# epeters13/pyCuSDR

Hardware: AMD Instinct MI355X
Metric: IQ Msamples/sec through Doppler matched-filter bank (256 bins, 2^20 chunk) (higher is better)
Workload: dtype f32

## Files before the change

__graft_entry__.py:

```python
import os
import subprocess
import sys

ROOT = os.path.dirname(os.path.abspath(__file__))
if ROOT not in sys.path:
    sys.path.insert(0, ROOT)

SRC = os.path.join(ROOT, 'pycusdr_amd', 'csrc', 'mfbank.hip')
CSRC = os.path.join(ROOT, 'pycusdr_amd', 'csrc')
DEPS = [SRC] + sorted(os.path.join(CSRC, h) for h in os.listdir(CSRC) if h.endswith(('.hpp', '.h'))) + [os.path.join(ROOT, 'include', 'mfbank.h')]
LIB = os.path.join(ROOT, 'pycusdr_amd', 'libmfbank.so')


HASHFILE = LIB + '.srchash'


def _src_hash():
    import hashlib
    h = hashlib.sha256()
    for d in DEPS:
        h.update(open(d, 'rb').read())
    return h.hexdigest()


def _stale():
    if not os.path.exists(LIB):
        return True
    try:
        return open(HASHFILE).read().strip() != _src_hash()
    except OSError:
        return True


def build(force=False):
    if force or _stale():
        import fcntl
        with open(LIB + '.lock', 'w') as lock:
            fcntl.flock(lock, fcntl.LOCK_EX)
            if force or _stale():
                hipcc = os.environ.get('HIPCC', '/opt/rocm/bin/hipcc')
                tmp = f'{LIB}.tmp.{os.getpid()}'
                cmd = [hipcc, '--offload-arch=gfx950', '-O3', '-std=c++17', '-shared', '-fPIC', '-pthread',
                       '-Wall', '-Wextra', '-Wno-unused-parameter', '-o', tmp, SRC]
                print('[build]', ' '.join(cmd), flush=True)
                subprocess.check_call(cmd, cwd=ROOT)
                os.replace(tmp, LIB)
                with open(HASHFILE, 'w') as f:
                    f.write(_src_hash())
    import pycusdr_amd
    from pycusdr_amd import _lib
    _lib.load()
    return LIB


def smoke():
    import numpy as np
    build()
    from pycusdr_amd import config as cfg, signals as sg
    from pycusdr_amd.protocol import loadProtocol
    from pycusdr_amd.demodulator import UHF
    from oracle import mfbank_oracle as orc

    bs, ov = 15, 1 << 10
    N = 1 << bs
    conf = cfg.bench_config('bench_GMSK', blockSize=bs, doppCarrierSteps=32)
    proto = loadProtocol('bench_GMSK')(conf=conf)
    demod = UHF.Demodulator(conf, proto, 'UHF-H')
    sig = sg.s1_stream(2, N, ov, 'GMSK', snr_db=20.0, seed=1)
    raw = demod.get_signalBufferHostPointer()
    raw[:] = sig[(N - ov):(N - ov) + N]
    fo, metric, _, snr = demod.uploadAndFindCarrier(raw)
    scores = demod.bank.get_scores()
    X = demod.bank.get_spectrum()
    bits, centres, trust, spSym = demod.demodulate()

    _, masks = proto.get_filter(N, 16, 3)
    ref = orc.doppler_scores(X, masks, demod.doppCyperSymNorm, True)
    rel = np.abs(scores - ref).max() / ref.max()
    assert rel < 1e-5, f'doppler scores differ from the oracle: {rel}'
    oidx, _ = orc.find_doppler_est(scores, demod.num_dopplers, 0, True)
    pick = orc.interpolate_doppler(oidx, demod.doppCyperSymNorm, demod.doppHzLUT, demod.centreFreqOffset)
    assert pick['dopplerIdxlast'] == int(demod.dopplerIdxlast) == N // 4, (pick, demod.dopplerIdxlast)
    xc = demod.bank.get_xcorr()
    ref_xc = orc.demod_xcorr(X, masks, int(demod.dopplerIdxlast))
    assert np.abs(xc - ref_xc).max() / np.abs(ref_xc).max() < 1e-5
    assert abs(spSym - 16.0) < 0.01 and len(bits) > 1900
    step = N - ov
    win = demod.blockWindows(2)[0]
    win[:] = sig[:2 * step + ov]
    demod.beginBlocks(0, 2)
    (_, rec0), (est1, rec1) = demod.endBlocks(0)
    assert est1[0] == fo and est1[3] == snr and rec1['spSym'] == spSym, (est1, fo, snr)
    raw[:] = sig[step:step + N]
    demod.uploadAndFindCarrier(raw)
    one = demod.demodulateDevice()
    assert np.array_equal(rec1['symbols'], one['symbols']) and np.array_equal(rec1['centres'], one['centres'])
    print(f'[smoke] ok: freq offset {fo:.1f} Hz, metric {metric:.2f}, SNR {snr:.1f} dB, spSym {spSym:.4f}, '
          f'{len(bits)} bits, score rel err {rel:.2e}; a batch of two blocks equals the blocks one by one')
    demod.close()


if __name__ == '__main__':
    build(force='--force' in sys.argv)
    if '--smoke' in sys.argv:
        smoke()
```

pycusdr_amd/csrc/wrap_kernels.hpp:

```cpp
#pragma once
#include "seg_kernels.hpp"

typedef _Float16 seg_h8 __attribute__((ext_vector_type(8)));
typedef float seg_f4 __attribute__((ext_vector_type(4)));

struct SegWArgs {
    SegFArgs f;
    const u32x4 *Wb;
    const int *Wexp;
    int T;
};

template <int PV, int KT>
struct SegWCfg {
    static constexpr int L = 256, PPL = 16, NT = 16, CT = 4;
    static constexpr int RT = PPL - PV;
    static constexpr int ND = RT + KT - 1;
    static constexpr int OFF = 16 * KT - 1;
    static constexpr int WSTR = 16 * (RT + KT);
    static_assert(RT >= 1 && RT + KT <= PPL, "the window is the first RT and the last KT register slots of a lane");
    static constexpr int WAVES = 1;
    static constexpr size_t lds_bytes() {
        return (size_t)SegCfg<256>::LDS_ELEMS * sizeof(cf) + (size_t)(SegCfg<256>::BLOCK / 64) * CT * WSTR * sizeof(cf);
    }
};

template <int KT>
struct SegWBin {
    seg_h8 hi[KT], lo[KT];
    cf q[8];
};

template <int PV, int KT>
DEVI void segw_body(const SegWArgs &w, const int blk) {
    static_assert(MFB_FFT_FUSED, "the fused 256-point transform");
    using Cfg = SegCfg<256>;
    using WC = SegWCfg<PV, KT>;
    constexpr int L = 256, NT = Cfg::NT, CT = Cfg::CT, PPL = Cfg::PPL, RT = WC::RT, ND = WC::ND, OFF = WC::OFF, WSTR = WC::WSTR;
    static_assert(NT == WC::NT && CT == WC::CT && PPL == WC::PPL, "256-point geometry");
    const SegFArgs &a = w.f;
    extern __shared__ __attribute__((aligned(16))) cf lds[];
    const int tid = threadIdx.x;
    const int wave = __builtin_amdgcn_readfirstlane(tid >> 6);
    const int lane = tid & 63;
    const int g = lane % NT;
    const int col = lane / NT;
    cf *mylds = lds + wave * Cfg::LDS_PER_TEAM + col * padlen(L);
    cf *wlds = lds + Cfg::LDS_ELEMS + wave * CT * WSTR;
    F256Regs f256;
    f256_setup(f256, a.twL + L, g);

    const int grp = blk % a.nsg;
    const int u = (blk / a.nsg) * (Cfg::BLOCK / 64) + wave;
    const int per_sc = a.nblk * a.nbc;
    const int sc = u / per_sc, rest = u - sc * per_sc;
    const int bk = rest / a.nbc, bc = rest - bk * a.nbc;
    const int gs0 = a.gbins ? 0 : (int)((long long)grp * a.nslots / a.nsg);
    const int glen = a.gbins ? a.nslots : (int)((long long)(grp + 1) * a.nslots / a.nsg) - gs0;
    const int gb0 = a.gbins ? (int)((long long)grp * a.dper / a.nsg) : 0;
    const int gblen = a.gbins ? (int)((long long)(grp + 1) * a.dper / a.nsg) - gb0 : a.dper;
    const int s0 = __builtin_amdgcn_readfirstlane(a.slot0 + gs0 + sc * a.fs);
    const int s1 = __builtin_amdgcn_readfirstlane(min(a.slot0 + gs0 + glen, s0 + a.fs));
    const int jb0 = __builtin_amdgcn_readfirstlane(gb0 + bc * a.fb);
    const int jb1 = __builtin_amdgcn_readfirstlane(min(gb0 + gblen, jb0 + a.fb));
    if (sc >= a.nsc || s0 >= s1 || jb0 >= jb1 || bk >= a.nblk) return;

    const unsigned nmask = (unsigned)a.N - 1u;
    const auto xr = mk_rsrc(a.x + (size_t)bk * (size_t)a.xstride, (unsigned)a.N * sizeof(cf));
    const auto qr = mk_rsrc(a.Qs, (unsigned)a.dper * (unsigned)(L * sizeof(float)));
    const auto br = mk_rsrc(w.Wb, (unsigned)a.dper * (unsigned)(KT * 2 * 64 * 16));
    auto load_q = [&](cf (&dst)[PPL / 2], int bin) {
#pragma unroll
        for (int jj = 0; jj < PPL / 4; ++jj)
            buf_load_cf2(qr, g * 4 * (int)sizeof(float), bin * (L * (int)sizeof(float)) + jj * NT * 4 * (int)sizeof(float), dst[2 * jj], dst[2 * jj + 1]);
    };
    auto load_b = [&](seg_h8 (&hi)[KT], seg_h8 (&lo)[KT], int bin) {
#pragma unroll
        for (int kk = 0; kk < KT; ++kk) {
            hi[kk] = __builtin_bit_cast(seg_h8, __builtin_amdgcn_raw_buffer_load_b128(br, lane * 16, (bin * KT + kk) * 2 * 1024, 0));
            lo[kk] = __builtin_bit_cast(seg_h8, __builtin_amdgcn_raw_buffer_load_b128(br, lane * 16, ((bin * KT + kk) * 2 + 1) * 1024, 0));
        }
    };
    constexpr int so_x = NT * (int)sizeof(cf);
    const int T = w.T;
    const int i16 = lane & 15, q = lane >> 4;
    const bool im_half = q >= 2;
    const int qo = 8 * (q & 1);

    const bool one_chunk = jb1 - jb0 <= 64;
    int wexl = jb0 + lane < jb1 ? w.Wexp[jb0 + lane] : 0;

    for (int slot = s0; slot < s1; ++slot) {
        cf v[PPL];
        {
            const unsigned e0 = (unsigned)(slot * CT + col) * (unsigned)a.V + (unsigned)g;
            const unsigned last = (unsigned)(slot * CT + CT - 1) * (unsigned)a.V + (unsigned)L;
            if (__builtin_amdgcn_readfirstlane(last <= (unsigned)a.N ? 1 : 0)) {
                const int vo_x = (int)(e0 * sizeof(cf));
#pragma unroll
                for (int i = 0; i < PPL; ++i) {
                    const cf t = buf_load_cf(xr, vo_x, i * so_x);
                    v[i] = mkc(t.y, t.x);
                }
            } else {
#pragma unroll
                for (int i = 0; i < PPL; ++i) {
                    const cf t = buf_load_cf(xr, (int)(((e0 + (unsigned)(NT * i)) & nmask) * sizeof(cf)), 0);
                    v[i] = mkc(t.y, t.x);
                }
            }
        }
        int ea;
        {
            cf *myw = wlds + col * WSTR;
            float mx = 0.f;
#pragma unroll
            for (int i = 0; i < RT; ++i) {
                const cf s = mkc(v[i].y, v[i].x);
                myw[g + NT * i + OFF] = s;
                mx = fmaxf(mx, fmaxf(fabsf(s.x), fabsf(s.y)));
            }
#pragma unroll
            for (int i = PPL - KT; i < PPL; ++i) {
                const int t = g + NT * i - L;
                const cf s = t >= -(T - 1) ? mkc(v[i].y, v[i].x) : mkc(0.f, 0.f);
                if (t + OFF >= 0) myw[t + OFF] = s;
                mx = fmaxf(mx, fmaxf(fabsf(s.x), fabsf(s.y)));
            }
#pragma unroll
            for (int m = 1; m < NT; m <<= 1) mx = fmaxf(mx, __shfl_xor(mx, m));
            int e;
            (void)frexpf(mx, &e);
            ea = 15 - e;
        }
        xsync<1>();
        cf A[PPL];
        {
            auto keep = [&](int, cf val, auto, auto nu) { A[decltype(nu)::value / NT] = val; };
            fft256_fused<0, PPL>(v, mylds, g, f256, keep);
        }
        cf pp[PPL / 2];
#pragma unroll
        for (int j = 0; j < PPL / 2; ++j) {
            const cf p0 = A[2 * j] * A[2 * j], p1 = A[2 * j + 1] * A[2 * j + 1];
            pp[j] = mkc(p0.x + p0.y, p1.x + p1.y);
        }
        seg_h8 ahi[CT][ND], alo[CT][ND];
        int eseg[CT];
#pragma unroll
        for (int c = 0; c < CT; ++c) {
            eseg[c] = __builtin_amdgcn_readlane(ea, NT * c);
            const cf *wc = wlds + c * WSTR;
#pragma unroll
            for (int di = 0; di < ND; ++di) {
                const int base = 16 * (di - (KT - 1)) + i16 - qo + OFF;
#pragma unroll
                for (int j = 0; j < 8; ++j) {
                    const cf s = wc[base - j];
                    const float sv = __builtin_ldexpf(im_half ? s.y : s.x, eseg[c]);
                    const _Float16 h = (_Float16)sv;
                    ahi[c][di][j] = h;
                    alo[c][di][j] = (_Float16)(sv - (float)h);
                }
            }
        }
        xsync<1>();

        for (int jc = jb0; jc < jb1; jc += 64) {
            if (!one_chunk) {
                wexl = jc + lane < jb1 ? w.Wexp[jc + lane] : 0;
                __builtin_amdgcn_s_waitcnt(0x0F70);
            }
            const int jc1 = min(jb1, jc + 64);
            SegWBin<KT> b0, b1;
            seg_f4 acc0[CT][RT], acc1[CT][RT];
            auto parseval = [&](const SegWBin<KT> &b) {
                cf t2[2] = {mkc(0.f, 0.f), mkc(0.f, 0.f)};
#pragma unroll
                for (int j = 0; j < PPL / 2; ++j) t2[j & 1] = __builtin_elementwise_fma(pp[j], b.q[j], t2[j & 1]);
                return (t2[0].x + t2[0].y) + (t2[1].x + t2[1].y);
            };
            auto fetch = [&](SegWBin<KT> &b, int bin) {
                load_q(b.q, bin);
                load_b(b.hi, b.lo, bin);
            };
            auto products = [&](seg_f4 (&acc)[CT][RT], const SegWBin<KT> &b) {
#pragma unroll
                for (int c = 0; c < CT; ++c) {
#pragma unroll
                    for (int rt = 0; rt < RT; ++rt) {
                        seg_f4 t = {0.f, 0.f, 0.f, 0.f};
#pragma unroll
                        for (int kk = 0; kk < KT; ++kk) {
                            const int di = rt - kk + KT - 1;
                            t = __builtin_amdgcn_mfma_f32_16x16x32_f16(alo[c][di], b.hi[kk], t, 0, 0, 0);
                            t = __builtin_amdgcn_mfma_f32_16x16x32_f16(ahi[c][di], b.lo[kk], t, 0, 0, 0);
                            t = __builtin_amdgcn_mfma_f32_16x16x32_f16(ahi[c][di], b.hi[kk], t, 0, 0, 0);
                        }
                        acc[c][rt] = t;
                    }
                }
            };
            auto finish = [&](const seg_f4 (&acc)[CT][RT], float tot, int jb) {
                const int wexp = __builtin_amdgcn_readlane(wexl, jb - jc);
                float wacc = 0.f;
#pragma unroll
                for (int c = 0; c < CT; ++c) {
                    float sq[RT];
#pragma unroll
                    for (int rt = 0; rt < RT; ++rt) {
                        const seg_f4 t = acc[c][rt];
                        sq[rt] = __builtin_fmaf(t.x, t.x, t.y * t.y) + __builtin_fmaf(t.z, t.z, t.w * t.w);
                    }
                    float s = sq[0];
#pragma unroll
                    for (int rt = 1; rt < RT; ++rt) s += sq[rt];
                    wacc += __builtin_ldexpf(s, wexp - 2 * eseg[c]);
                }
                float sv = __builtin_fmaf((float)L, tot, -wacc);
                sv += __int_as_float(__builtin_amdgcn_mov_dpp(__float_as_int(sv), 0xB1, 0xF, 0xF, true));
                sv += __int_as_float(__builtin_amdgcn_mov_dpp(__float_as_int(sv), 0x4E, 0xF, 0xF, true));
                sv += __int_as_float(__builtin_amdgcn_mov_dpp(__float_as_int(sv), 0x124, 0xF, 0xF, true));
                sv += __int_as_float(__builtin_amdgcn_mov_dpp(__float_as_int(sv), 0x128, 0xF, 0xF, true));
                const float r0 = __int_as_float(__builtin_amdgcn_readlane(__float_as_int(sv), 0));
                const float r1 = __int_as_float(__builtin_amdgcn_readlane(__float_as_int(sv), 16));
                const float r2 = __int_as_float(__builtin_amdgcn_readlane(__float_as_int(sv), 32));
                const float r3 = __int_as_float(__builtin_amdgcn_readlane(__float_as_int(sv), 48));
                return (r0 + r1) + (r2 + r3);
            };
            auto store = [&](float total, int jb) {
                if (lane < a.MU)
                    a.partials[((size_t)(a.part_row0 + bk * a.dper + jb) * a.MU + lane) * a.parts + slot] = lane == 0 ? total * a.scale : 0.f;
            };
            auto step = [&](seg_f4 (&accn)[CT][RT], SegWBin<KT> &bn, const seg_f4 (&accp)[CT][RT], SegWBin<KT> &bp, float totp, int jb) {
                const float totn = parseval(bn);
                fetch(bp, min(jb + 2, jc1 - 1));
                products(accn, bn);
                const float total = finish(accp, totp, jb);
#pragma unroll
                for (int i = 0; i < CT * RT * KT * 3; ++i) {
                    __builtin_amdgcn_sched_group_barrier(0x8, 1, 0);
                    __builtin_amdgcn_sched_group_barrier(0x2, 2, 0);
                }
                store(total, jb);
                return totn;
            };
            fetch(b0, jc);
            fetch(b1, min(jc + 1, jc1 - 1));
            float tot0 = parseval(b0), tot1 = 0.f;
            products(acc0, b0);
            int jb = jc;
            while (true) {
                if (jb + 1 >= jc1) {
                    store(finish(acc0, tot0, jb), jb);
                    break;
                }
                tot1 = step(acc1, b1, acc0, b0, tot0, jb);
                ++jb;
                if (jb + 1 >= jc1) {
                    store(finish(acc1, tot1, jb), jb);
                    break;
                }
                tot0 = step(acc0, b0, acc1, b1, tot1, jb);
                ++jb;
            }
        }
    }
}
template <int PV, int KT>
__global__ void __launch_bounds__(SegCfg<256>::BLOCK) __attribute__((amdgpu_waves_per_eu(SegWCfg<PV, KT>::WAVES, SegWCfg<PV, KT>::WAVES)))
k_segw(SegWArgs w) {
    segw_body<PV, KT>(w, (int)blockIdx.x);
}
```

Measured before the change: 2342.

## Defer partial stores via buffer stores and retune MFMA interleave schedule

The per-bin result store now goes through a raw buffer resource with a scalar row offset. It is deferred by one step so it issues at the start of the next step instead of after the MFMA block. Buffer loads are restructured so bin offsets become scalar offsets, and the Parseval accumulation is split into scalar FMAs. Empty asm constraints pin the MFMA operands into AGPRs, backed by a new compiler flag for the VGPR-form MFMA. The sched_group_barrier pattern is rewritten to interleave loads, stores, DS and VALU ops with the MFMAs differently, which risks register pressure or scheduling regressions.

```diff
diff --git a/__graft_entry__.py b/__graft_entry__.py
--- a/__graft_entry__.py
+++ b/__graft_entry__.py
@@ -40,7 +40,7 @@
             if force or _stale():
                 hipcc = os.environ.get('HIPCC', '/opt/rocm/bin/hipcc')
                 tmp = f'{LIB}.tmp.{os.getpid()}'
-                cmd = [hipcc, '--offload-arch=gfx950', '-O3', '-std=c++17', '-shared', '-fPIC', '-pthread',
+                cmd = [hipcc, '--offload-arch=gfx950', '-O3', '-std=c++17', '-mllvm', '-amdgpu-mfma-vgpr-form', '-shared', '-fPIC', '-pthread',
                        '-Wall', '-Wextra', '-Wno-unused-parameter', '-o', tmp, SRC]
                 print('[build]', ' '.join(cmd), flush=True)
                 subprocess.check_call(cmd, cwd=ROOT)
diff --git a/pycusdr_amd/csrc/wrap_kernels.hpp b/pycusdr_amd/csrc/wrap_kernels.hpp
--- a/pycusdr_amd/csrc/wrap_kernels.hpp
+++ b/pycusdr_amd/csrc/wrap_kernels.hpp
@@ -69,16 +69,16 @@
     const auto xr = mk_rsrc(a.x + (size_t)bk * (size_t)a.xstride, (unsigned)a.N * sizeof(cf));
     const auto qr = mk_rsrc(a.Qs, (unsigned)a.dper * (unsigned)(L * sizeof(float)));
     const auto br = mk_rsrc(w.Wb, (unsigned)a.dper * (unsigned)(KT * 2 * 64 * 16));
-    auto load_q = [&](cf (&dst)[PPL / 2], int bin) {
+    auto load_q = [&](cf (&dst)[PPL / 2], int so) {
 #pragma unroll
         for (int jj = 0; jj < PPL / 4; ++jj)
-            buf_load_cf2(qr, g * 4 * (int)sizeof(float), bin * (L * (int)sizeof(float)) + jj * NT * 4 * (int)sizeof(float), dst[2 * jj], dst[2 * jj + 1]);
+            buf_load_cf2(qr, g * 4 * (int)sizeof(float) + jj * NT * 4 * (int)sizeof(float), so, dst[2 * jj], dst[2 * jj + 1]);
     };
-    auto load_b = [&](seg_h8 (&hi)[KT], seg_h8 (&lo)[KT], int bin) {
+    auto load_b = [&](seg_h8 (&hi)[KT], seg_h8 (&lo)[KT], int so) {
 #pragma unroll
         for (int kk = 0; kk < KT; ++kk) {
-            hi[kk] = __builtin_bit_cast(seg_h8, __builtin_amdgcn_raw_buffer_load_b128(br, lane * 16, (bin * KT + kk) * 2 * 1024, 0));
-            lo[kk] = __builtin_bit_cast(seg_h8, __builtin_amdgcn_raw_buffer_load_b128(br, lane * 16, ((bin * KT + kk) * 2 + 1) * 1024, 0));
+            hi[kk] = __builtin_bit_cast(seg_h8, __builtin_amdgcn_raw_buffer_load_b128(br, lane * 16 + kk * 2 * 1024, so, 0));
+            lo[kk] = __builtin_bit_cast(seg_h8, __builtin_amdgcn_raw_buffer_load_b128(br, lane * 16 + (kk * 2 + 1) * 1024, so, 0));
         }
     };
     constexpr int so_x = NT * (int)sizeof(cf);
@@ -89,6 +89,8 @@
 
     const bool one_chunk = jb1 - jb0 <= 64;
     int wexl = jb0 + lane < jb1 ? w.Wexp[jb0 + lane] : 0;
+    const int pstep = __builtin_amdgcn_readfirstlane(a.MU * a.parts * (int)sizeof(float));
+    const int pvo = lane < a.MU ? lane * a.parts * (int)sizeof(float) : 0x7FFFFFFF;
 
     for (int slot = s0; slot < s1; ++slot) {
         cf v[PPL];
@@ -162,6 +164,8 @@
                     ahi[c][di][j] = h;
                     alo[c][di][j] = (_Float16)(sv - (float)h);
                 }
+                asm("" : "+a"(ahi[c][di]));
+                asm("" : "+a"(alo[c][di]));
             }
         }
         xsync<1>();
@@ -172,19 +176,30 @@
                 __builtin_amdgcn_s_waitcnt(0x0F70);
             }
             const int jc1 = min(jb1, jc + 64);
+            const auto pr = mk_rsrc(a.partials + ((size_t)(a.part_row0 + bk * a.dper + jc) * a.MU) * a.parts + slot, 64u * (unsigned)pstep);
             SegWBin<KT> b0, b1;
             seg_f4 acc0[CT][RT], acc1[CT][RT];
+            unsigned pend = 0u;
+            int pendvo = 0x7FFFFFFF;
             auto parseval = [&](const SegWBin<KT> &b) {
-                cf t2[2] = {mkc(0.f, 0.f), mkc(0.f, 0.f)};
-#pragma unroll
-                for (int j = 0; j < PPL / 2; ++j) t2[j & 1] = __builtin_elementwise_fma(pp[j], b.q[j], t2[j & 1]);
-                return (t2[0].x + t2[0].y) + (t2[1].x + t2[1].y);
+                float tx[2] = {0.f, 0.f}, ty[2] = {0.f, 0.f};
+#pragma unroll
+                for (int j = 0; j < PPL / 2; ++j) {
+                    tx[j & 1] = __builtin_fmaf(pp[j].x, b.q[j].x, tx[j & 1]);
+                    ty[j & 1] = __builtin_fmaf(pp[j].y, b.q[j].y, ty[j & 1]);
+                    asm("" : "+v"(tx[j & 1]), "+v"(ty[j & 1]));
+                }
+                float s0 = tx[0] + ty[0];
+                asm("" : "+v"(s0));
+                return s0 + (tx[1] + ty[1]);
             };
             auto fetch = [&](SegWBin<KT> &b, int bin) {
-                load_q(b.q, bin);
-                load_b(b.hi, b.lo, bin);
-            };
-            auto products = [&](seg_f4 (&acc)[CT][RT], const SegWBin<KT> &b) {
+                load_b(b.hi, b.lo, bin * (KT * 2 * 1024));
+                load_q(b.q, bin * (L * (int)sizeof(float)));
+            };
+            auto products = [&](seg_f4 (&acc)[CT][RT], SegWBin<KT> &b) {
+#pragma unroll
+                for (int kk = 0; kk < KT; ++kk) asm("" : "+a"(b.hi[kk]), "+a"(b.lo[kk]));
 #pragma unroll
                 for (int c = 0; c < CT; ++c) {
 #pragma unroll
@@ -211,6 +226,7 @@
                     for (int rt = 0; rt < RT; ++rt) {
                         const seg_f4 t = acc[c][rt];
                         sq[rt] = __builtin_fmaf(t.x, t.x, t.y * t.y) + __builtin_fmaf(t.z, t.z, t.w * t.w);
+                        asm("" : "+v"(sq[rt]));
                     }
                     float s = sq[0];
 #pragma unroll
@@ -226,23 +242,40 @@
                 const float r1 = __int_as_float(__builtin_amdgcn_readlane(__float_as_int(sv), 16));
                 const float r2 = __int_as_float(__builtin_amdgcn_readlane(__float_as_int(sv), 32));
                 const float r3 = __int_as_float(__builtin_amdgcn_readlane(__float_as_int(sv), 48));
-                return (r0 + r1) + (r2 + r3);
-            };
-            auto store = [&](float total, int jb) {
-                if (lane < a.MU)
-                    a.partials[((size_t)(a.part_row0 + bk * a.dper + jb) * a.MU + lane) * a.parts + slot] = lane == 0 ? total * a.scale : 0.f;
-            };
+                float r01 = r0 + r1;
+                asm("" : "+v"(r01));
+                return r01 + (r2 + r3);
+            };
+            auto row = [&](float total) { return lane == 0 ? __float_as_uint(total * a.scale) : 0u; };
+            auto store = [&](unsigned val, int vo, int so) { __builtin_amdgcn_raw_buffer_store_b32(val, pr, vo, so, 0); };
+            auto row_off = [&](int jb) { return __builtin_amdgcn_readfirstlane(max(jb - jc, 0)) * pstep; };
             auto step = [&](seg_f4 (&accn)[CT][RT], SegWBin<KT> &bn, const seg_f4 (&accp)[CT][RT], SegWBin<KT> &bp, float totp, int jb) {
-                const float totn = parseval(bn);
+                store(pend, pendvo, row_off(jb - 1));
                 fetch(bp, min(jb + 2, jc1 - 1));
                 products(accn, bn);
                 const float total = finish(accp, totp, jb);
+                const float totn = parseval(bn);
+                pend = row(total);
+                pendvo = pvo;
 #pragma unroll
                 for (int i = 0; i < CT * RT * KT * 3; ++i) {
                     __builtin_amdgcn_sched_group_barrier(0x8, 1, 0);
-                    __builtin_amdgcn_sched_group_barrier(0x2, 2, 0);
-                }
-                store(total, jb);
+                    if (i < 4) {
+                        if (i == 2) {
+                            __builtin_amdgcn_sched_group_barrier(0x40, 1, 0);
+                            __builtin_amdgcn_sched_group_barrier(0x4, 1, 0);
+                        } else {
+                            __builtin_amdgcn_sched_group_barrier(0x4, 2, 0);
+                        }
+                    } else if (i < 14) {
+                        __builtin_amdgcn_sched_group_barrier(0x20, 1, 0);
+                        __builtin_amdgcn_sched_group_barrier(0x6, 1, 0);
+                    } else if ((i & 3) && i < 96) {
+                        __builtin_amdgcn_sched_group_barrier(0x6, 1, 0);
+                    } else {
+                        __builtin_amdgcn_sched_group_barrier(0x6, 2, 0);
+                    }
+                }
                 return totn;
             };
             fetch(b0, jc);
@@ -252,13 +285,15 @@
             int jb = jc;
             while (true) {
                 if (jb + 1 >= jc1) {
-                    store(finish(acc0, tot0, jb), jb);
+                    store(pend, pendvo, row_off(jb - 1));
+                    store(row(finish(acc0, tot0, jb)), pvo, row_off(jb));
                     break;
                 }
                 tot1 = step(acc1, b1, acc0, b0, tot0, jb);
                 ++jb;
                 if (jb + 1 >= jc1) {
-                    store(finish(acc1, tot1, jb), jb);
+                    store(pend, pendvo, row_off(jb - 1));
+                    store(row(finish(acc1, tot1, jb)), pvo, row_off(jb));
                     break;
                 }
                 tot0 = step(acc0, b0, acc1, b1, tot1, jb);
```

Result: faster. 2575 (median of 6 runs) (+10.0%).
